# simplew4y/VeritasFi

Hardware: AMD Instinct MI355X
Metric: queries/sec top-100 over 10Mx768 corpus (higher is better)
Workload: dtype f16

## Files before the change

### veritasfi_amd/csrc/vf_api.hip

```cpp
#include "../../include/veritasfi_hip.h"
#include "vf_internal.h"
#include "vf_route.h"

#include <fcntl.h>
#include <float.h>
#include <sys/stat.h>
#include <unistd.h>
#include <math.h>
#include <string.h>

#include <algorithm>
#include <atomic>
#include <mutex>
#include <string>
#include <vector>

using namespace vf;

static thread_local std::string g_err;

static int fail(int code, const std::string& msg) {
    g_err = msg;
    return code;
}
// ... 106 lines not shown
    int nq = 0, k = 0;
    int64_t* d_ids = nullptr; float* d_scores = nullptr;
    hipStream_t user = nullptr;
};

}

struct vf_index {
    int device = 0;
    int64_t n = 0;
    int64_t cap = 0;
    int d = 0, dp = 0, dtype = 0;
    int64_t id_offset = 0;
    int n_cu = 256;
    int64_t aux_applied = -1;
    bool owns_rows = false;
    void* rows_orig = nullptr;
    void* rows_scan = nullptr;
    bool owns_scan = false;
    float* norm = nullptr;
    float* inv_scan = nullptr;
    float* cn_cache = nullptr;
    unsigned char* rows_img = nullptr;
    bool owns_img = false;
    float* inv_img = nullptr;
    float rho_max = 0.0f;
    float rho_mean = 0.0f;
    bool image_refused = false;
    float rho_sum = 0.0f;
    std::mutex mu;
    Slot slots[kSlots];
    int64_t force_path = -1, sample_rows = -1, margin = -1, cap_opt = 0, waves_opt = 0, scan_g = 0,
            refresh_every = 128, debug = 0, steal_opt = 0, wide_opt = 1, wide_sync = -1, wide_mfma = -1, wide8_waves = 8, wide8_stage = 0,
            aux_cus = -1, sample_grid = -1, overlap_scans = -1, scan_impl = 2, sample_impl = -1, scan_image = 1, wide_rows = 1, image_mfma = -1;
    vf_search_stats stats{};
    bool profile = false;
    double prof_scan_ms = 0.0, prof_pipe_ms = 0.0;
    int64_t prof_launches = 0, prof_bytes = 0;
    hipEvent_t ev_span = nullptr;
    bool span_started = false;
    bool span_slot[4] = {false, false, false, false};
    DevBuf st_q, st_ids, st_sc;
    DevBuf st_add, st_rho;
    std::vector<vf_index*> shards;
    std::vector<int> peer_ok;
    GroupSlot gslots[kSlots];
};

static int ensure_pinned(Slot& s, size_t nq_total) {
    if (nq_total <= s.h_cap) return VF_OK;
    if (s.h_flags) (void)hipHostFree(s.h_flags);
    if (s.h_counts) (void)hipHostFree(s.h_counts);
    s.h_flags = nullptr; s.h_counts = nullptr; s.h_cap = 0;
    size_t cap = std::max<size_t>(nq_total, 256);
    VF_HIP(hipHostMalloc((void**)&s.h_flags, cap * sizeof(int), hipHostMallocMapped));
    VF_HIP(hipHostMalloc((void**)&s.h_counts, cap * sizeof(u32), hipHostMallocMapped));
    VF_HIP(hipHostGetDevicePointer((void**)&s.d_flags, s.h_flags, 0));
    VF_HIP(hipHostGetDevicePointer((void**)&s.d_counts, s.h_counts, 0));
    s.h_cap = cap;
    return VF_OK;
}

static int build_image(vf_index* ix, int64_t mode);

static bool known_dtype(int64_t dtype) { return dtype >= VF_DTYPE_F32 && dtype <= VF_DTYPE_INT8; }
static size_t dtype_bytes(int dtype) { return dtype == VF_DTYPE_F32 ? 4 : (dtype == VF_DTYPE_F16 ? 2 : 1); }

static RouteIn route_in(const vf_index* ix, const Slot* s = nullptr) {
    RouteIn in;
    in.n = ix->n; in.d = ix->d; in.dp = ix->dp; in.dtype = ix->dtype; in.n_cu = ix->n_cu;
    in.has_scan = ix->rows_scan && ix->inv_scan;
    in.has_image = ix->rows_img != nullptr; in.rho_mean = ix->rho_mean;
    in.group = !ix->shards.empty();
    in.aux_applied = ix->aux_applied;
    in.masked = s && s->scan_stream && s->scan_stream != s->stream;
    in.force_path = ix->force_path; in.wide = ix->wide_opt; in.wide_mfma = ix->wide_mfma; in.wide8_waves = ix->wide8_waves;
    in.wide8_stage = ix->wide8_stage; in.wide_rows = ix->wide_rows; in.scan_impl = ix->scan_impl; in.sample_impl = ix->sample_impl;
    in.sample_grid = ix->sample_grid; in.steal = ix->steal_opt; in.scan_image = ix->scan_image; in.image_mfma = ix->image_mfma;
    in.aux_cus = ix->aux_cus; in.overlap_scans = ix->overlap_scans; in.margin = ix->margin; in.cap = ix->cap_opt; in.waves = ix->waves_opt;
    in.sample_rows = ix->sample_rows; in.debug = ix->debug;
    return in;
}

static int build_common(vf_index* ix) {
    hipDeviceProp_t prop;
    VF_HIP(hipGetDeviceProperties(&prop, ix->device));
    ix->n_cu = prop.multiProcessorCount > 0 ? prop.multiProcessorCount : 256;
    VF_HIP(scan_configure());
    const int dt = ix->dtype;
    const size_t scan_esz = byte_rows(dt) ? 1 : 2;
    ix->dp = (ix->d + 127) / 128 * 128;
    ix->cap = ix->n;
    const size_t npad = (size_t)ix->cap + 64;
    VF_HIP(hipMalloc((void**)&ix->norm, npad * sizeof(float)));
    VF_HIP(hipMalloc((void**)&ix->inv_scan, npad * sizeof(float)));
    VF_HIP(hipMemset(ix->norm, 0, npad * sizeof(float)));
    VF_HIP(hipMemset(ix->inv_scan, 0, npad * sizeof(float)));
    const bool need_scan = ix->n > kSmallN;
    void* scan_out = nullptr;
    if (need_scan) {
        if (dt != VF_DTYPE_F32 && ix->dp == ix->d && ((uintptr_t)ix->rows_orig % 16) == 0) {
            ix->rows_scan = ix->rows_orig;
            ix->owns_scan = false;
        } else {
            VF_HIP(hipMalloc((void**)&ix->rows_scan, (size_t)ix->cap * ix->dp * scan_esz));
            ix->owns_scan = true;
            scan_out = ix->rows_scan;
        }
    }
    VF_HIP(launch_prep_rows(ix->rows_orig, dt, ix->n, ix->d, ix->dp, scan_out, ix->norm, ix->inv_scan, nullptr));
    VF_TRY(build_image(ix, ix->scan_image));
    if (ix->n > 0 && ix->n <= kSmallN) {
        VF_HIP(hipMalloc((void**)&ix->cn_cache, (size_t)std::min<int64_t>(ix->cap, kSmallN) * ix->d * sizeof(float)));
// ... 574 lines not shown
    else if (s == "wide8_waves") {
#ifdef VF_EXPERIMENTS
        if (value != 4 && value != 8) return fail(VF_EINVAL, "wide8_waves must be 8 (one 512-thread workgroup per CU, 256-query tiles: the default) or 4 (two 256-thread workgroups, 128-query tiles: measured slower, DESIGN.md 4)");
#else
        if (value != 8) return fail(VF_EINVAL, "wide8_waves must be 8 (the 4-wave form was measured slower and is built with -DVF_EXPERIMENTS only: DESIGN.md 4)");
#endif
        ix->wide8_waves = value;
    }
    else if (s == "wide_mfma") { if (!in_range(-1, 1)) return fail(VF_EINVAL, "wide_mfma must be -1 (auto: the fp8 instruction for e4m3 rows), 0 (fp16 matrix instruction on converted rows) or 1 (the fp8 instruction on the e4m3 row bytes: k_scan_wide8)"); ix->wide_mfma = value; }
    else if (s == "wide_sync") { if (!in_range(-1, 8)) return fail(VF_EINVAL, "wide_sync must be -1 (off) or a slack of 0..8 super-tiles"); ix->wide_sync = value; }
    else if (s == "aux_cus") {
        if (!in_range(-1, 128)) return fail(VF_EINVAL, "aux_cus must be -1 (auto) or in [0, 128]");
        if (ix->aux_applied >= 0 && value != ix->aux_cus)
            return fail(VF_EINVAL, "aux_cus is fixed once the first search has created the scan streams: set it before searching");
        ix->aux_cus = value;
    }
    else if (s == "sample_grid") { if (!in_range(-1, 1024)) return fail(VF_EINVAL, "sample_grid must be -1 (auto), 0 (one workgroup per range) or a workgroup count"); ix->sample_grid = value; }
    else if (s == "scan_impl") { if (!in_range(1, 5)) return fail(VF_EINVAL, "scan_impl must be 1 (k_scan), 2 (auto: k_scan2 for fp16 rows, k_scan2r where it measured faster), 3 (k_scan2 wherever it fits, e4m3 rows converted), 4 (k_scan2 for fp16 rows, never k_scan2r) or 5 (k_scan2r wherever a shape of it exists: fp16 rows of 384 / 512 / 768 / 1024 elements, e4m3 rows of 768 / 1024)"); ix->scan_impl = value; }
    else if (s == "sample_impl") { if (!in_range(-1, 1)) return fail(VF_EINVAL, "sample_impl must be -1 (auto: k_scan2r's operand path for the sample pass where it exists and the CU split is on), 0 (k_scan) or 1 (k_scan2r wherever it fits)"); ix->sample_impl = value; }
    else if (s == "overlap_scans") { if (!in_range(-1, 1)) return fail(VF_EINVAL, "overlap_scans must be -1 (auto), 0 or 1"); ix->overlap_scans = value; }
    else if (s == "scan_image") {
        if (!in_range(0, 2)) return fail(VF_EINVAL, "scan_image must be 0 (off), 1 (auto: when it fits with headroom) or 2 (force)");
        if (!ix->shards.empty()) { ix->scan_image = value; return VF_OK; }
        for (const Slot& sl : ix->slots) if (sl.pending) return fail(VF_EINVAL, "scan_image cannot change while a search is pending");
        DeviceGuard restore_callers_device;
        VF_HIP(hipSetDevice(ix->device));
        VF_HIP(hipDeviceSynchronize());
        ix->image_refused = false;
        if (value == 0) free_image(ix);
        else VF_TRY(build_image(ix, value));
        ix->scan_image = value;
    }
    else if (s == "image_mfma") { if (!in_range(-1, 2)) return fail(VF_EINVAL, "image_mfma must be -1 (auto), 0 (the int8 row image on the fp16 matrix instruction, fp16 queries), 1 (on the int8 matrix instruction, the queries as one int8 plane) or 2 (as two planes, hi + lo: the band of 0)"); ix->image_mfma = value; }
    else if (s == "wide_rows") { if (!in_range(0, 2)) return fail(VF_EINVAL, std::string("wide_rows must be 0 (rows of more than 2432 padded elements never take the fused path), 1 (auto: from ") + std::to_string(kWideRowsMinRows) + " rows, e4m3 rows from " + std::to_string(kWideRowsMinRows8) + ", int8 rows from " + std::to_string(kWideRowsMinRowsI8) + ") or 2 (wherever k_scan_ksplit / k_scan_ksplit8 serve them; int8 rows: from " + std::to_string(kWideRowsMinRowsI8) + " rows)"); ix->wide_rows = value; }
    else if (s == "debug") ix->debug = value;
    else if (s == "profile") {
        ix->profile = value != 0; ix->prof_scan_ms = ix->prof_pipe_ms = 0.0; ix->prof_launches = 0;
        ix->span_started = false;
        for (bool& b : ix->span_slot) b = false;
    }
    else return fail(VF_EINVAL, "vf_index_set_option: unknown option " + s);
    return VF_OK;
}

static int exact_search(vf_index* ix, Slot& s, const float* qn_dev, int nq, int k, int64_t* out_ids,
                        float* out_scores, hipStream_t st) {
    const int dt = ix->dtype;
    const int64_t chunk = kSmallN;
    const int64_t nchunks = ix->n == 0 ? 1 : (ix->n + chunk - 1) / chunk;
    if (nchunks > 1) {
        int64_t P = 1;
        while (P < 2 * (int64_t)k) P <<= 1;
        if (P * 8 > 160 * 1024) return fail(VF_EUNSUPPORTED, "exact chunked search supports k <= 8192 when n > 16384");
    }
    VF_TRY(s.dense_s.ensure((size_t)nq * chunk * sizeof(float)));
    if (nchunks == 1) {
        const float* cn = ix->cn_cache;
        if (!cn && ix->n > 0) {
            VF_TRY(s.cn_tmp.ensure((size_t)chunk * ix->d * sizeof(float)));
            VF_HIP(launch_normalize_rows(ix->rows_orig, dt, 0, ix->n, ix->d, ix->norm, s.cn_tmp.as<float>(), st));
            cn = s.cn_tmp.as<float>();
        }
        VF_HIP(launch_dense_dot16(qn_dev, nq, cn, ix->n, ix->d, s.dense_s.as<float>(), chunk, st));
        VF_HIP(launch_sort_rows(s.dense_s.as<float>(), chunk, nq, (int)ix->n, k, ix->id_offset, (long long*)out_ids,
                                out_scores, k, st));
        return VF_OK;
// ... 168 lines not shown
        s.timed = ix->profile;
        if (s.timed) VF_HIP(hipEventRecord(s.ev_t[2], st));
        for (int b0 = 0; b0 < nq; b0 += bl) {
            const int nb = std::min(bl, nq - b0);
            VF_TRY(wide_pass(ix, s, in, p, d_queries + (size_t)b0 * ix->d, nb, k, d_ids + (size_t)b0 * k, d_scores + (size_t)b0 * k,
                             b0, s.qn.as<float>() + (size_t)b0 * ix->d, s.timed && b0 == 0, st, slot_id));
            ++s.wide_launches; s.wide_queries += nb;
        }
        if (s.timed) VF_HIP(hipEventRecord(s.ev_t[3], st));
        VF_HIP(hipEventRecord(s.ev_done, st));
        return VF_OK;
    }
    VF_TRY(s.s0.ensure((size_t)kMaxBatch * p.total_waves * p.samp * sizeof(float)));
    VF_TRY(s.cnt.ensure((size_t)kMaxBatch * kCntStride * sizeof(u32)));
    VF_TRY(s.tau.ensure(kMaxBatch * sizeof(int)));
    VF_TRY(s.hist.ensure((size_t)kMaxBatch * kHistBins * sizeof(u32)));
    VF_TRY(s.hist_coarse.ensure((size_t)kMaxBatch * 64 * sizeof(u32)));
    VF_TRY(s.cand.ensure((size_t)kMaxBatch * p.cap * sizeof(u64)));
    VF_TRY(s.tilecnt.ensure((size_t)p.grid * sizeof(u32)));
    s.timed = ix->profile;
    if (s.timed) VF_HIP(hipEventRecord(s.ev_t[2], st));
    if (s.wgbase_n != ix->n || s.wgbase_grid != p.grid) {
        std::vector<long long> base(p.grid);
        for (int w = 0; w < p.grid; ++w) base[w] = ix->n * (long long)w / p.grid;
        VF_TRY(s.wgbase.ensure((size_t)p.grid * sizeof(long long)));
        VF_HIP(hipMemcpy(s.wgbase.p, base.data(), (size_t)p.grid * sizeof(long long), hipMemcpyHostToDevice));
        s.wgbase_n = ix->n; s.wgbase_grid = p.grid;
    }
    for (int b0 = 0; b0 < nq; b0 += bl) {
        const int nb = std::min(bl, nq - b0);
        const BatchRoute b = route_batch(in, r, nb);
        const int qt = b.tile;
        float* qn_b = s.qn.as<float>() + (size_t)b0 * ix->d;
        VF_HIP(launch_prep_queries(d_queries + (size_t)b0 * ix->d, nb, ix->d, ix->dp, qt, qn_b, s.image_i8 ? nullptr : s.qimg.as<_Float16>(), st));
        ScanArgs a{};
        a.rows = (const char*)ix->rows_scan; a.inv_scan = ix->inv_scan; a.qimg = s.qimg.as<_Float16>();
        if (s.image_i8) {
            VF_TRY(s.qimg8.ensure((size_t)ix->dp * kMaxBatch * 2));
            VF_TRY(s.epsq.ensure(kMaxBatch * sizeof(float)));
            VF_TRY(s.qscale.ensure(kMaxBatch * sizeof(float)));
            VF_TRY(s.bandq.ensure(2 * kMaxBatch * sizeof(int)));
            VF_HIP(launch_prep_q8(qn_b, nb, ix->d, ix->dp, qt, s.image_i8, (signed char*)s.qimg8.p, s.qscale.as<float>(), s.epsq.as<float>(), s.bandq.as<int>(),
                                  p.eps, p.tau_band, p.fine_band, st));
            a.qimg = (const _Float16*)s.qimg8.p; a.q_scale = s.qscale.as<float>(); a.band_q = s.bandq.as<int>();
        }
        a.n = ix->n; a.dp = ix->dp; a.row_bytes = (long long)ix->dp * (byte_rows(ix->dtype) ? 1 : 2); a.total_waves = p.total_waves; a.samp = p.samp;
        if (p.image) { a.rows = (const char*)ix->rows_img; a.inv_scan = ix->inv_img; a.off_scan = image_offsets(ix); a.row_bytes = ix->dp; }
        a.s0 = s.s0.as<float>(); a.wg_base = s.wgbase.as<long long>(); a.cnt = s.cnt.as<u32>(); a.tau_bin = s.tau.as<int>(); a.hist = s.hist.as<u32>();
        a.cand = s.cand.as<u64>(); a.cap = p.cap; a.kprime = p.kprime; a.tau_band = p.tau_band;
        a.hist_coarse = s.hist_coarse.as<u32>(); a.stage_cap = b.stage_cap;
        a.tile_cnt = ix->steal_opt ? s.tilecnt.as<u32>() : nullptr; a.scan_grid = p.grid;
        a.dbg = nullptr;
        if (ix->debug & 128) { VF_TRY(s.dbg.ensure((size_t)p.total_waves * ((ix->debug & 512) ? 72 : 4) * sizeof(u64))); a.dbg = s.dbg.as<u64>(); if (ix->debug & 512) VF_HIP(hipMemsetAsync(s.dbg.p, 0, s.dbg.bytes, st)); }
        a.refresh_every = (int)std::min<int64_t>(256, std::max<int64_t>(4, std::max<int64_t>(1, ix->refresh_every) * nb / kMaxBatch));
        while (a.refresh_every & (a.refresh_every - 1)) a.refresh_every &= a.refresh_every - 1;
        a.nq = nb; a.debug = (int)ix->debug;
        if (ix->n / p.total_waves < p.samp)
            VF_HIP(hipMemsetAsync(a.s0, 0xFF, (size_t)qt * p.total_waves * p.samp * sizeof(float), st));
        switch (b.sample) {
        case kKernelKsplit: VF_HIP(launch_scan_ksplit(a, kModeSample, b.sample_grid, st)); break;
        case kKernelKsplit8: VF_HIP(launch_scan_ksplit8(a, kModeSample, b.sample_grid, b.sample_rows, st)); break;
        case kKernelScan2r: {
            ScanArgs as = a;
            as.stage_cap = 0;
            VF_HIP(launch_scan2r_sample(as, qt, b.sample_grid, b.sample_rows, st));
            break;
        }
        default: VF_HIP(launch_scan(a, kModeSample, qt, b.sample_grid, (int)ix->scan_g, b.sample_rows, st));
        }
        VF_HIP(launch_sel0(a, qt, st));
        hipStream_t sst = s.scan_stream;
        if (sst != st) {
            VF_HIP(hipEventRecord(s.ev_pro, st));
            VF_HIP(hipStreamWaitEvent(sst, s.ev_pro, 0));
        }
        if (!route_overlap(in))
// ... 790 lines not shown
```

### veritasfi_amd/csrc/vf_internal.h

```cpp
#pragma once
#include <hip/hip_runtime.h>
#include <math.h>
#include <stdint.h>

#include "../../include/veritasfi_hip.h"

#include <string>

#include "vf_ksplit_geom.h"

namespace vf {

int set_error(int code, const std::string& msg);

typedef unsigned long long u64;
typedef unsigned int u32;

struct DeviceGuard {
    int prev = -1;
    DeviceGuard() { if (hipGetDevice(&prev) != hipSuccess) prev = -1; }
    ~DeviceGuard() { if (prev >= 0) (void)hipSetDevice(prev); }
    DeviceGuard(const DeviceGuard&) = delete;
    DeviceGuard& operator=(const DeviceGuard&) = delete;
};
// ... 109 lines not shown
    unsigned char* img;
    float* inv_img; float* off_img;
    u32* rho_max_bits; float* rho_sum;
};
hipError_t launch_append_rows(const AppendArgs& a, hipStream_t s);
hipError_t launch_prep_queries(const float* q, int nq, int d, int dp, int qn_tile ,
                               float* qn, _Float16* qimg, hipStream_t s);
hipError_t launch_normalize_rows(const void* rows, int dt , long long row0, long long nrows, int d,
                                 const float* norm, float* out, hipStream_t s);
hipError_t launch_normalize_rows_gather(const void* rows, int dt, const long long* sel , int nsel, int d,
                                        const float* norm, float* out, hipStream_t s);
hipError_t launch_dense_dot16(const float* qn, int nq, const float* cn, long long nrows, int d,
                              float* out, long long out_stride, hipStream_t s);
hipError_t launch_sort_rows(const float* scores, long long score_stride, int nq, int n, int k,
                            long long id_base, long long* out_ids, float* out_scores, int out_stride,
                            hipStream_t s);
hipError_t launch_scan(const ScanArgs& a, int mode, int qn_tile, int grid, int want_g ,
                       RowForm rows , hipStream_t s);
hipError_t launch_rebias_i8(const void* in, void* out, long long bytes, hipStream_t s);
hipError_t launch_debug_cvt_e4m3(const unsigned char* in, float* out, int count, hipStream_t s);
hipError_t launch_debug_mfma_i8(const signed char* A, const signed char* B, int* C, hipStream_t s);
hipError_t launch_scan2(const ScanArgs& a, int qn_tile, int grid, RowForm rows , hipStream_t s);
hipError_t launch_scan2r(const ScanArgs& a, int qn_tile, int grid, RowForm rows, hipStream_t s);
hipError_t launch_scan2r_sample(const ScanArgs& a, int qn_tile, int grid, RowForm rows, hipStream_t s);
hipError_t launch_scan_ksplit(const ScanArgs& a, int mode, int grid, hipStream_t s);
hipError_t launch_scan_ksplit8(const ScanArgs& a, int mode, int grid, RowForm rows, hipStream_t s);
hipError_t launch_scan_wide(const ScanArgs& a, int mode, RowForm rows , hipStream_t s);
hipError_t launch_prep_wide8(const float* qn, int nq, int d, int dp, int qtot, unsigned char* img8, float* eps_q, hipStream_t s);
hipError_t launch_scan_wide8(const ScanArgs& a, int waves , hipStream_t s);
int scan_wide8_occupancy(int waves, int stage_cap);
hipError_t launch_prep_q8(const float* qn, int nq, int d, int dp, int qn_tile, int planes , signed char* img8, float* q_scale, float* eps_q, int* band_q,
                          float eps_img, int tau_band, int fine_band, hipStream_t s);
hipError_t launch_sel0(const ScanArgs& a, int qn_tile, hipStream_t s);
hipError_t launch_final(FinalArgs a, int nq, hipStream_t s);
hipError_t launch_merge_topk(const long long* ids_parts, const float* score_parts, int nparts, int nq,
                             int k, long long* ids, float* scores, hipStream_t s);
hipError_t launch_merge_topk_packed(const void* parts, int nparts, int nq, int k, long long* ids, float* scores,
                                    hipStream_t s);
hipError_t launch_fuse_rank(const float* a, const float* b, int n, float* out, long long* order,
                            hipStream_t s);
inline long long packed_part_bytes(int nq, int k) { return ((long long)nq * k * 12 + 15) / 16 * 16; }
hipError_t scan_configure();

}
```

### veritasfi_amd/csrc/vf_kernels.hip

```cpp
#include "vf_internal.h"

#include <float.h>
#include <algorithm>
#include <type_traits>

#include <mutex>

namespace vf {

typedef _Float16 h8 __attribute__((ext_vector_type(8)));
typedef _Float16 h4 __attribute__((ext_vector_type(4)));
typedef float f16v __attribute__((ext_vector_type(16)));
typedef int i4v __attribute__((ext_vector_type(4)));
typedef int i16v __attribute__((ext_vector_type(16)));
typedef int i8v __attribute__((ext_vector_type(8)));

__device__ __forceinline__ float group16_tree(float acc) {
    acc = acc + __shfl_down(acc, 8, 16);
    acc = acc + __shfl_down(acc, 4, 16);
    acc = acc + __shfl_down(acc, 2, 16);
    acc = acc + __shfl_down(acc, 1, 16);
    return acc;
}

// ... 211 lines not shown
    const int slot = blockIdx.x;
    const int tid = threadIdx.x;
    if (slot < nq) {
        const float* x = q + (long long)slot * d;
        for (int j = tid; j < d; j += 256) xs[j] = x[j];
        __syncthreads();
        if (tid < 16) {
            float acc = 0.0f;
            for (int j = tid; j < d; j += 16) acc = __builtin_fmaf(xs[j], xs[j], acc);
            acc = group16_tree(acc);
            if (tid == 0) s_norm = canon_norm_from_sumsq(acc);
        }
        __syncthreads();
        const float inv = canon_inv(s_norm);
        for (int j = tid; j < dp; j += 256) {
            float v = 0.0f;
            if (j < d) {
                v = xs[j] * inv;
                qn[(long long)slot * d + j] = v;
            }
            if (qimg) qimg[((long long)(j >> 3) * QN + slot) * 8 + (j & 7)] = (_Float16)v;
        }
    } else if (qimg) {
        for (int j = tid; j < dp; j += 256) qimg[((long long)(j >> 3) * QN + slot) * 8 + (j & 7)] = (_Float16)0.0f;
    }
}

hipError_t launch_prep_queries(const float* q, int nq, int d, int dp, int qn_tile, float* qn, _Float16* qimg,
                               hipStream_t s) {
    hipLaunchKernelGGL(k_prep_queries, dim3(qn_tile), dim3(256), (size_t)d * sizeof(float), s, q, nq, d, dp, qn_tile, qn, qimg);
    return hipGetLastError();
}

__global__ __launch_bounds__(256) void k_prep_q8(const float* qn, int nq, int d, int dp, int QN, int planes, signed char* img8, float* q_scale,
                                                  float* eps_q, int* band_q, float eps_img, int tau_band, int fine_band) {
    __shared__ float red_f[256];
    __shared__ double red_d[256];
    const int slot = blockIdx.x, tid = threadIdx.x;
    const bool live = slot < nq;
    float mx = 0.0f;
    if (live) for (int j = tid; j < d; j += 256) mx = fmaxf(mx, fabsf(qn[(long long)slot * d + j]));
    red_f[tid] = mx;
    __syncthreads();
    for (int o = 128; o; o >>= 1) { if (tid < o) red_f[tid] = fmaxf(red_f[tid], red_f[tid + o]); __syncthreads(); }
    mx = red_f[0];
    bool finite = mx <= FLT_MAX;
    const float sc = (finite && mx > 0.0f) ? mx / 127.0f : 1.0f;
    const float sc2 = sc / 254.0f;
    double res = 0.0;
    for (int j = tid; j < dp; j += 256) {
        float code = 0.0f, lo = 0.0f;
        if (live && j < d) {
            const float x = qn[(long long)slot * d + j];
            code = fminf(fmaxf(rintf(x / sc), -127.0f), 127.0f);
            double dx = (double)x - (double)sc * (double)code;
            if (planes == 2) {
                lo = fminf(fmaxf(rintf((float)dx / sc2), -127.0f), 127.0f);
                dx -= (double)sc2 * (double)lo;
            }
            res += dx * dx;
        }
        const long long at = (((long long)(j >> 4) * planes) * QN + slot) * 16 + (j & 15);
        img8[at] = (signed char)(int)code;
        if (planes == 2) img8[at + (long long)QN * 16] = (signed char)(int)lo;
    }
    red_d[tid] = res;
    __syncthreads();
    for (int o = 128; o; o >>= 1) { if (tid < o) red_d[tid] += red_d[tid + o]; __syncthreads(); }
    if (tid == 0) {
        const double rd = sqrt(red_d[0]);
        float rho = (float)rd;
        if ((double)rho < rd) rho = nextafterf(rho, INFINITY);
        if (!finite || !(rd <= (double)FLT_MAX)) rho = INFINITY;
        const Q8Bound b = image_q8_bound(live ? rho : 0.0f);
        q_scale[slot] = live ? (planes == 2 ? sc2 : sc) : 0.0f;
        eps_q[slot] = image_q8_eps(eps_img, b.eps_add);
        band_q[slot] = tau_band + b.tau_bins;
        band_q[QN + slot] = fine_band + b.fine_bins;
    }
}

hipError_t launch_prep_q8(const float* qn, int nq, int d, int dp, int qn_tile, int planes, signed char* img8, float* q_scale, float* eps_q, int* band_q,
                          float eps_img, int tau_band, int fine_band, hipStream_t s) {
    hipLaunchKernelGGL(k_prep_q8, dim3(qn_tile), dim3(256), 0, s, qn, nq, d, dp, qn_tile, planes, img8, q_scale, eps_q, band_q, eps_img, tau_band, fine_band);
    return hipGetLastError();
}

__device__ __forceinline__ float normalised_elem(float x, float nm) { return x * canon_inv(nm); }

__global__ __launch_bounds__(256) void k_normalize_rows(const void* rows, int dt, long long row0,
                                                         long long nrows, int d, const float* norm, float* out) {
    const long long total = nrows * (long long)d;
    for (long long i = (long long)blockIdx.x * 256 + threadIdx.x; i < total; i += (long long)gridDim.x * 256) {
        const long long r = i / d;
        out[i] = normalised_elem(load_elem(rows, dt, (row0 + r) * (long long)d + (i - r * d)), norm[row0 + r]);
    }
}

hipError_t launch_normalize_rows(const void* rows, int dt, long long row0, long long nrows, int d,
                                 const float* norm, float* out, hipStream_t s) {
    if (nrows <= 0) return hipSuccess;
    long long blocks = (nrows * (long long)d + 255) / 256;
    if (blocks > 65536) blocks = 65536;
    hipLaunchKernelGGL(k_normalize_rows, dim3((unsigned)blocks), dim3(256), 0, s, rows, dt, row0, nrows, d, norm,
                       out);
    return hipGetLastError();
}

__global__ __launch_bounds__(256) void k_append_rows(AppendArgs a) {
    __shared__ u32 wg_max;
    __shared__ float wg_sum;
    const bool stats = a.img != nullptr;
// ... 1828 lines not shown
                        if constexpr (PLANES == 2) { v = v * 254.0f + (float)acci[1][nt][e]; acci[1][nt][e] = 0; }
                        acc[nt][e] = v * sq[nt];
                        acci[0][nt][e] = 0;
                    }
            }
            epi.sync_tau = sync_now;
            if (sync_now) {
#pragma unroll
                for (int nt = 0; nt < NT; ++nt) epi.tau_g[nt] = *(const int*)(sc + (nt * kQueryTile + r31) * 4);
            }
            tile_epilogue<NT, MODE, true, true, F8 >= 2>(a, acc, epi, t0, t_hi, t_s0, lane, ctl);
#pragma unroll
            for (int nt = 0; nt < NT; ++nt)
#pragma unroll
                for (int e = 0; e < 16; ++e) acc[nt][e] = 0.0f;
            VF_PC(pt1 = cyc(); pc_epi += pt1 - pt0)
            ++tiles_done;
            if (!more) break;
            cur_tile = nxt;
            src_cur = src_nxt;
        }
    }
    if (dbg && dbg_rec > 4) dbg[69] = (unsigned long long)tiles_done;
    asm volatile("s_waitcnt vmcnt(0)" ::: "memory");
    if (MODE == kModeSample) return;
    if (lane == 0) atomicAdd((u32*)(ctl + 8), 1u);
    if (dbg) dbg[1] = wall_clock64();
    __syncthreads();
    if (dbg) dbg[2] = wall_clock64();
    {
        const u32 staged = *(const u32*)ctl;
        const u32 nst = staged < (u32)a.stage_cap ? staged : (u32)a.stage_cap;
        uint4* ent = (uint4*)(ctl + kCtlBytes);
        u32* qcnt = (u32*)(kImgBytes ? img : smem);
        u32* qbase = qcnt + QN;
        if (tid < QN) qcnt[tid] = 0u;
        __syncthreads();
        for (u32 i = tid; i < nst; i += THREADS) {
            const uint4 e = ent[i];
            const u32 q = e.z & 0xFFu;
            if (e.w != 1u || q >= (u32)QN) continue;
            ent[i].w = 2u + atomicAdd(qcnt + q, 1u);
        }
        __syncthreads();
        if (tid < QN) {
            const u32 c = qcnt[tid];
            qbase[tid] = c ? atomicAdd(a.cnt + tid * kCntStride, c) : 0u;
        }
        __syncthreads();
        for (u32 i = tid; i < nst; i += THREADS) {
            const uint4 e = ent[i];
            if (e.w < 2u) continue;
            const u32 q = e.z & 0xFFu;
            const u32 gs = qbase[q] + (e.w - 2u);
            if (gs < (u32)a.cap) a.cand[(long long)q * a.cap + gs] = ((u64)e.y << 32) | (u64)e.x;
        }
    }
    if (dbg && dbg_rec > 4) dbg[71] = __builtin_amdgcn_s_memtime() - c_entry;
#ifdef VF_EXPERIMENTS
    if (dbg && dbg_rec > 4 && prof) { dbg[4] = pc_wait; dbg[5] = pc_use; dbg[6] = pc_fill; dbg[7] = pc_head; dbg[8] = pc_epi; dbg[9] = pc_n; }
#endif
#undef VF_PC
    if (dbg) dbg[3] = wall_clock64();
}

constexpr int kWideNT = kWideQ / kQueryTile, kWideRows = 256;
// ... 1065 lines not shown
        if (rows_are_fp8) hipLaunchKernelGGL((k_scan2<1, 1>), dim3(grid), dim3(kScan2Threads), lds, s, a);
        else hipLaunchKernelGGL((k_scan2<1, 0>), dim3(grid), dim3(kScan2Threads), lds, s, a);
    } else {
        if (rows_are_fp8) hipLaunchKernelGGL((k_scan2<2, 1>), dim3(grid), dim3(kScan2Threads), lds, s, a);
        else hipLaunchKernelGGL((k_scan2<2, 0>), dim3(grid), dim3(kScan2Threads), lds, s, a);
    }
    return hipGetLastError();
}

#define VF_SCAN2R_PRODUCT(X, NT, MODE) X(NT, MODE, 0, 12, 6, 6, 1) X(NT, MODE, 0, 16, 6, 4, 1) X(NT, MODE, 0, 8, 4, 6, 1) X(NT, MODE, 0, 6, 3, 6, 1) X(NT, MODE, 1, 6, 3, 6, 1) X(NT, MODE, 1, 8, 3, 4, 1) \
    X(NT, MODE, 2, 6, 3, 6, 1) X(NT, MODE, 3, 6, 6, 6, 1) X(NT, MODE, 4, 6, 3, 6, 1)
#ifdef VF_EXPERIMENTS
#define VF_SCAN2R_SHAPES(X, NT, MODE) VF_SCAN2R_PRODUCT(X, NT, MODE) X(NT, MODE, 0, 12, 6, 6, 0) X(NT, MODE, 1, 6, 3, 4, 1)
#else
#define VF_SCAN2R_SHAPES(X, NT, MODE) VF_SCAN2R_PRODUCT(X, NT, MODE)
#endif
#define VF_SCAN2R_ALL(X) VF_SCAN2R_SHAPES(X, 1, kModeMain) VF_SCAN2R_SHAPES(X, 2, kModeMain) VF_SCAN2R_SHAPES(X, 1, kModeSample) VF_SCAN2R_SHAPES(X, 2, kModeSample)
static hipError_t launch_scan2r_any(const ScanArgs& a, int qn_tile, int mode, int grid, RowForm f8, size_t lds, hipStream_t s) {
    Scan2rShape sh = scan2r_shape(a.dp, f8);
#ifdef VF_EXPERIMENTS
    if (f8 == 1 && a.dp == 768 && (a.debug & 2048)) sh.RING = 4;
#endif
    const int nt = qn_tile / kQueryTile;
    bool done = false;
    const int ar = (!f8 && a.dp == 768 && (a.debug & 1024)) ? 0 : 1;
#define VF_X(NT, MODE, F8, S_, RB_, RING_, AR_) \
    if (!done && nt == NT && mode == MODE && f8 == F8 && sh.S == S_ && sh.RB == RB_ && sh.RING == RING_ && ar == AR_) { \
        hipLaunchKernelGGL((k_scan2r<NT, MODE, F8, S_, RB_, RING_, AR_>), dim3(grid), dim3(kScan2Waves * 64), lds, s, a); done = true; }
    VF_SCAN2R_ALL(VF_X)
#undef VF_X
    return done ? hipGetLastError() : hipErrorInvalidValue;
}
hipError_t launch_scan2r(const ScanArgs& a, int qn_tile, int grid, RowForm f8, hipStream_t s) {
    return launch_scan2r_any(a, qn_tile, kModeMain, grid, f8, scan2r_lds_bytes(a.dp, qn_tile, a.stage_cap, f8), s);
}
hipError_t launch_scan2r_sample(const ScanArgs& a, int qn_tile, int grid, RowForm f8, hipStream_t s) {
    return launch_scan2r_any(a, qn_tile, kModeSample, grid, f8, scan2r_lds_bytes(a.dp, qn_tile, 0, f8), s);
}

template <int NT, int G, int MODE>
static hipError_t configure_one() {
    hipError_t e = hipFuncSetAttribute((const void*)k_scan<NT, G, MODE, 0>, hipFuncAttributeMaxDynamicSharedMemorySize,
                                       160 * 1024);
    if (e != hipSuccess) return e;
    e = hipFuncSetAttribute((const void*)k_scan<NT, G, MODE, 2>, hipFuncAttributeMaxDynamicSharedMemorySize, 160 * 1024);
    if (e != hipSuccess) return e;
    return hipFuncSetAttribute((const void*)k_scan<NT, G, MODE, 1>, hipFuncAttributeMaxDynamicSharedMemorySize, 160 * 1024);
}

__device__ __forceinline__ int wave_tau_from_lds(const u32* lh, int kprime, int lane) {
    u32 hv[32];
    u32 sum = 0;
#pragma unroll
    for (int i = 0; i < 32; ++i) { hv[i] = lh[lane * 32 + i]; sum += hv[i]; }
    u32 suf = sum;
#pragma unroll
    for (int off = 1; off < 64; off <<= 1) {
        const u32 v = __shfl_down(suf, off);
        if (lane + off < 64) suf += v;
    }
    const u32 above = suf - sum;
    int best = -1;
    if (above < (u32)kprime && suf >= (u32)kprime) {
        u32 run = above;
        bool found = false;
#pragma unroll
// ... 457 lines not shown
```

### veritasfi_amd/csrc/vf_route.h

```cpp
#pragma once
#include <math.h>
#include <stdint.h>

#include <algorithm>

#include "../../include/veritasfi_hip.h"
#include "vf_ksplit_geom.h"

namespace vf {

struct RouteIn {
    int64_t n = 0;
    int d = 0, dp = 0, dtype = 0, n_cu = 256;
    bool has_scan = false;
    bool has_image = false;
    float rho_mean = 0.0f;
    bool group = false;
    int64_t aux_applied = -1;
    bool masked = false;
    int64_t force_path = -1, wide = 1, wide_mfma = -1, wide8_waves = 8, wide8_stage = 0, wide_rows = 1, scan_impl = 2, sample_impl = -1,
            sample_grid = -1, steal = 0, scan_image = 1, image_mfma = -1, aux_cus = -1, overlap_scans = -1, margin = -1, cap = 0, waves = 0,
            sample_rows = -1, debug = 0;
};

enum ScanKernel : int {
    kKernelNone = 0, kKernelScan = 1, kKernelScan2 = 2, kKernelWide = 3, kKernelWide8 = 4, kKernelScan2r = 5, kKernelKsplit = 6,
    kKernelKsplit8 = 7,
};

struct FusedPlan {
    int kprime, cap, total_waves, grid, samp;
    float eps;
    bool image;
    int tau_band, fine_band;
};

struct SearchRoute {
    int path = 2;
    int per_pass = kMaxBatch;
    bool wide = false;
    bool image = false;
    int planes = 0;
    FusedPlan plan{};
};

struct BatchRoute {
    int tile;
    ScanKernel sample;
    int sample_grid;
    RowForm sample_rows;
    ScanKernel main;
    RowForm main_rows;
    int stage_cap;
};

// ... 99 lines not shown
    int margin = in.margin >= 0 ? (int)in.margin : std::max(24, k / 4);
    const double u16 = 1.0 / 2048.0;
    const float eps_plan = (float)(u16 * (in.dtype == VF_DTYPE_F32 ? 2.0 : 1.0) + sqrt((double)in.d) * ldexp(1.0, -24) +
                                   2.0 * in.d * ldexp(1.0, -24) + 1e-6);
    if (in.margin < 0 && ksplit_width(in.dp)) {
        const double z = sqrt(2.0 * log(std::max(3.0, (double)in.n / k)));
        margin = std::max(margin, (int)ceil(2.5 * eps_plan * k * z * sqrt((double)in.d)));
    }
    p.kprime = in.margin >= 0 ? k + margin : (k + margin + 31) / 32 * 32;
    p.kprime = std::min(p.kprime, 4096);
    int cap = kMaxCap;
    while (cap < 4 * p.kprime && cap < 16384) cap <<= 1;
    if (in.cap > 0) { cap = 1; while (cap < in.cap) cap <<= 1; cap = std::min(cap, 16384); }
    while (cap < 2 * p.kprime) cap <<= 1;
    p.cap = cap;
    const int64_t scan_cus = in.n_cu - route_aux_cus(in);
    int64_t wgs = std::min<int64_t>(scan_cus, std::max<int64_t>(1, in.n / 512));
    if (in.waves > 0) wgs = std::max<int64_t>(1, in.waves / (kScanThreads / 64));
    p.grid = (int)wgs;
    p.total_waves = p.grid * (kScanThreads / 64);
    p.samp = in.sample_rows > 0 ? (int)in.sample_rows : ((in.n <= 1500000 && 8ll * p.total_waves >= 16ll * p.kprime) ? 8 : 16);
    if (in.cap <= 0) {
        const double sample_rows = (double)p.total_waves * p.samp;
        const double expect = p.kprime * (1.0 + log(std::max(1.0, (double)in.n / std::max(1.0, sample_rows))));
        while (p.cap < (int)(1.6 * expect) && p.cap < 32768) p.cap <<= 1;
    }
    p.eps = eps_plan;
    if (image) {
        image_bound(in.d, in.dtype, in.rho_mean, &p.eps, &p.tau_band, &p.fine_band);
        p.kprime = k;
        p.cap = 32768;
    }
    return p;
}

constexpr int kWideMinQueries = 129;
constexpr int kWideMinQueries16 = 65;
constexpr int kWideMinQueriesKsplit = 33;
constexpr int kWideMinQueriesKsplit8 = 65;
constexpr int kWideMaxQueries = 1024;
constexpr int kWideTile = kWideQ;
inline bool wide_possible(const RouteIn& in, int nq) {
    const bool ks = ksplit_width(in.dp);
    if (in.wide == 0 || nq < (in.wide > 1 ? (int)in.wide : ks ? (byte_rows(in.dtype) ? kWideMinQueriesKsplit8 : kWideMinQueriesKsplit) : (byte_rows(in.dtype) ? kWideMinQueries : kWideMinQueries16))) return false;
    return in.dp % (byte_rows(in.dtype) ? 256 : 128) == 0;
}

inline WidePass route_wide_pass(const RouteIn& in, const FusedPlan& p, int nb) {
    WidePass w;
    w.qtot = (nb + kWideTile - 1) / kWideTile * kWideTile;
    w.jtiles = w.qtot / kWideTile;
    w.rgroups = std::max(1, in.n_cu / w.jtiles);
    w.cap = p.cap;
    if (p.kprime > 256) w.cap = std::max(w.cap, 16384);
    const bool w8 = (in.wide_mfma > 0 || (in.wide_mfma < 0 && !ksplit_width(in.dp))) && in.dtype == VF_DTYPE_FP8_E4M3 && in.dp % 64 == 0 &&
                    (in.n / w.rgroups + 2 * 256) * (int64_t)in.dp < (int64_t)0xFFFFFFFFll;
    if (w8) {
        if (p.kprime > 256) w.cap = std::max(w.cap, 32768);
    }
    w.main = w8 ? kKernelWide8 : kKernelWide;
    w.rows = stored_rows(in.dtype);
    w.samp = w.jtiles >= 2 ? 64 : 32;
    w.waves = in.wide8_waves == 4 ? 4 : 8;
    w.main_jtiles = w8 && w.waves == 4 ? (nb + 127) / 128 : w.jtiles;
    w.stage_cap = !w8 ? kWideStageCap
                      : in.wide8_stage > 0 ? (int)std::min<int64_t>(in.wide8_stage, scan_wide8_stage_cap(w.waves)) : scan_wide8_stage_cap(w.waves);
// ... 20 lines not shown
    const int qt = b.tile = qn_tile_for(nb);
    const bool ks = ksplit_width(in.dp);
    const int64_t steal = in.steal, scan_impl = in.scan_impl;
    const bool f8rows = in.dtype == VF_DTYPE_FP8_E4M3 || p.image;
    const bool i8conv = in.dtype == VF_DTYPE_INT8 && !p.image;
    const bool r_f8_auto = f8rows && scan_impl == 2 && in.n > kScan2rMinRows && !steal && scan2r_auto_width(in.dp, true);
    const bool sample_r = p.image || (!i8conv && in.sample_impl != 0 && scan_impl != 1 && scan2r_stage_cap(in.dp, qt, f8rows ? kRowsE4m3 : kRowsF16) >= kStageMinEntries &&
                          (in.sample_impl == 1 || (!f8rows && in.masked && scan2r_auto_width(in.dp, false)) || r_f8_auto));
    if (ks) {
        b.sample = byte_rows(in.dtype) ? kKernelKsplit8 : kKernelKsplit;
        b.sample_grid = p.grid;
        b.sample_rows = stored_rows(in.dtype);
    } else if (sample_r) {
        const int64_t sg_r = in.sample_grid > 0 ? in.sample_grid : (in.masked ? route_aux_cus(in) : p.grid);
        b.sample = kKernelScan2r;
        b.sample_grid = (int)std::min<int64_t>(std::max<int64_t>(sg_r, 1), p.grid);
        b.sample_rows = p.image ? image_rows(r.planes) : (f8rows ? kRowsE4m3 : kRowsF16);
    } else {
        const int64_t sg_opt = in.sample_grid >= 0 ? in.sample_grid : (in.masked ? 4 * route_aux_cus(in) : 0);
        b.sample = kKernelScan;
        b.sample_grid = sg_opt > 0 ? (int)std::min<int64_t>(sg_opt, p.grid) : p.grid;
        b.sample_rows = stored_rows(in.dtype);
    }
    const RowForm f8 = in.dtype == VF_DTYPE_FP8_E4M3 ? kRowsE4m3 : kRowsF16;
    if (ks) {
        b.main = byte_rows(in.dtype) ? kKernelKsplit8 : kKernelKsplit;
        b.main_rows = stored_rows(in.dtype);
        b.stage_cap = ksplit_stage_cap(in);
        return b;
    }
    if (p.image) {
        b.main = kKernelScan2r;
        b.main_rows = image_rows(r.planes);
        b.stage_cap = scan2r_stage_cap(in.dp, qt, b.main_rows);
        return b;
    }
    const int cap2 = i8conv ? 0 : (((scan_impl == 3 || ((scan_impl == 2 || scan_impl == 4 || scan_impl == 5) && !f8)) && !steal) ? scan2_stage_cap(in.dp, qt, f8) : 0);
    const bool r_auto = scan_impl == 2 && in.n > kScan2rMinRows && scan2r_auto_width(in.dp, f8 != 0) && (f8 || (in.masked && route_overlap(in)));
#ifdef VF_EXPERIMENTS
    const bool dbg_r = f8 || !(in.debug & (32 | 64));
#else
    const bool dbg_r = true;
#endif
    const int capr = ((scan_impl == 5 || r_auto) && !steal && dbg_r && !i8conv) ? scan2r_stage_cap(in.dp, qt, f8) : 0;
    if (capr >= kStageMinEntries) {
        b.main = kKernelScan2r; b.main_rows = f8; b.stage_cap = capr;
    } else if (cap2 >= kStageMinEntries) {
        b.main = kKernelScan2; b.main_rows = f8; b.stage_cap = cap2;
    } else {
        b.main = kKernelScan; b.main_rows = stored_rows(in.dtype); b.stage_cap = scan_stage_cap(in.dp, qt);
    }
    return b;
}

}
```

### veritasfi_amd/csrc/vf_scan_lds.h

```cpp
#pragma once
#include <stddef.h>

#if defined(__HIPCC__)
#define VF_HD __host__ __device__ __forceinline__
#else
#define VF_HD inline
#endif

namespace vf {

constexpr int kQueryTile = 32;
constexpr int kMaxBatch = 64;
constexpr int kRowTile = 32;
constexpr int kScanThreads = 512;
constexpr int kHistBins = 2048;
constexpr int kSmallN = 16384;
constexpr int kMaxCap = 8192;
constexpr int kCntStride = 32;
constexpr int kMaxKFused = 2048;

constexpr int kLdsBytes = 160 * 1024;
constexpr int kStageMaxBytes = 32 * 1024;
constexpr int kStageMinEntries = 256;

enum RowForm : int {
    kRowsF16 = 0,
    kRowsE4m3 = 1,
    kRowsI8 = 2,
    kRowsI8Mfma1 = 3,
    kRowsI8Mfma2 = 4,
};
VF_HD bool row_form_bytes(RowForm f) { return f != kRowsF16; }

constexpr int kCtlBytes = 272;

VF_HD int stage_entries(size_t fixed) {
    const size_t freeb = fixed < (size_t)kLdsBytes ? (size_t)kLdsBytes - fixed : 0;
    return (int)((freeb < (size_t)kStageMaxBytes ? freeb : (size_t)kStageMaxBytes) / 16);
}

VF_HD size_t scan_lds_bytes(int dp, int qn_tile) { return (size_t)dp * qn_tile * 2 + kCtlBytes; }
VF_HD int scan_stage_cap(int dp, int qn_tile) { return stage_entries(scan_lds_bytes(dp, qn_tile)); }

constexpr int kScan2Waves = 4, kRing = 3, kSegBytes = 4096, kScratchBytes = 1024;

VF_HD size_t scan2_lds_bytes(int dp, int qn_tile, int stage_cap) {
    const size_t img = (size_t)dp * qn_tile * 2;
    return img + (size_t)kScan2Waves * (kRing * kSegBytes + kScratchBytes) + kCtlBytes + (size_t)stage_cap * 16;
}
VF_HD int scan2_stage_cap(int dp, int qn_tile, RowForm rows) {
    const size_t fixed = scan2_lds_bytes(dp, qn_tile, 0);
    if ((dp >> (rows ? 7 : 6)) < kRing) return 0;
    if (fixed + kStageMinEntries * 16 > (size_t)kLdsBytes) return 0;
    return stage_entries(fixed);
}

struct Scan2rShape { int S, RB, RING; };
VF_HD Scan2rShape scan2r_shape(int dp, RowForm f8) {
    if (!f8 && dp == 768) return {12, 6, 6};
    if (!f8 && dp == 1024) return {16, 6, 4};
    if (!f8 && dp == 512) return {8, 4, 6};
    if (!f8 && dp == 384) return {6, 3, 6};
    if (f8 == kRowsI8Mfma1) return dp == 768 ? Scan2rShape{6, 6, 6} : Scan2rShape{0, 0, 0};
    if (f8 == kRowsI8Mfma2) return dp == 768 ? Scan2rShape{6, 3, 6} : Scan2rShape{0, 0, 0};
    if (f8 && dp == 768) return {6, 3, 6};
    if (f8 && dp == 1024) return {8, 3, 4};
    return {0, 0, 0};
}
VF_HD size_t scan2r_lds_bytes(int dp, int qn_tile, int stage_cap, RowForm f8) {
    const Scan2rShape sh = scan2r_shape(dp, f8);
    const size_t seg_img = (size_t)(f8 ? 128 : 64) * qn_tile * 2;
    return (size_t)(sh.S - sh.RB) * seg_img + (size_t)kScan2Waves * (sh.RING * kSegBytes + kScratchBytes) + kCtlBytes + (size_t)stage_cap * 16;
}
VF_HD int scan2r_stage_cap(int dp, int qn_tile, RowForm f8) {
    if (scan2r_shape(dp, f8).S == 0) return 0;
    const size_t fixed = scan2r_lds_bytes(dp, qn_tile, 0, f8);
    if (fixed + kStageMinEntries * 16 > (size_t)kLdsBytes) return 0;
    return stage_entries(fixed);
}

constexpr int kWideQ = 256, kWideKC = 64;
constexpr int kWideBuf = (kWideKC / 8) * kWideQ * 16;
constexpr int kWideCtl = 16 + 3 * kWideQ * 4;
constexpr int kWideStageCap = 3584;

VF_HD size_t scan_wide_lds_bytes(int stage_cap) { return (size_t)3 * kWideBuf + kWideCtl + (size_t)stage_cap * 16; }
VF_HD size_t scan_wide8_lds_bytes(int waves, int stage_cap) {
    return waves == 8 ? scan_wide_lds_bytes(stage_cap) : (size_t)65536 + (16 + 3 * 128 * 4) + (size_t)stage_cap * 16;
}
VF_HD int scan_wide8_stage_cap(int waves) { return waves == 8 ? kWideStageCap : 896; }

}
```

Measured before the change: 47970.

## Fuse query normalisation into int8 query prep and lift image-scan stage cap

```diff
diff --git a/veritasfi_amd/csrc/vf_api.hip b/veritasfi_amd/csrc/vf_api.hip
--- a/veritasfi_amd/csrc/vf_api.hip
+++ b/veritasfi_amd/csrc/vf_api.hip
@@ -162,7 +162,7 @@
     Slot slots[kSlots];
     int64_t force_path = -1, sample_rows = -1, margin = -1, cap_opt = 0, waves_opt = 0, scan_g = 0,
             refresh_every = 128, debug = 0, steal_opt = 0, wide_opt = 1, wide_sync = -1, wide_mfma = -1, wide8_waves = 8, wide8_stage = 0,
-            aux_cus = -1, sample_grid = -1, overlap_scans = -1, scan_impl = 2, sample_impl = -1, scan_image = 1, wide_rows = 1, image_mfma = -1;
+            aux_cus = -1, sample_grid = -1, overlap_scans = -1, scan_impl = 2, sample_impl = -1, scan_image = 1, wide_rows = 1, image_mfma = -1, image_stage = -1;
     vf_search_stats stats{};
     bool profile = false;
     double prof_scan_ms = 0.0, prof_pipe_ms = 0.0;
@@ -208,7 +208,7 @@
     in.wide8_stage = ix->wide8_stage; in.wide_rows = ix->wide_rows; in.scan_impl = ix->scan_impl; in.sample_impl = ix->sample_impl;
     in.sample_grid = ix->sample_grid; in.steal = ix->steal_opt; in.scan_image = ix->scan_image; in.image_mfma = ix->image_mfma;
     in.aux_cus = ix->aux_cus; in.overlap_scans = ix->overlap_scans; in.margin = ix->margin; in.cap = ix->cap_opt; in.waves = ix->waves_opt;
-    in.sample_rows = ix->sample_rows; in.debug = ix->debug;
+    in.sample_rows = ix->sample_rows; in.debug = ix->debug; in.image_stage = ix->image_stage;
     return in;
 }
 
@@ -849,6 +849,7 @@
         ix->scan_image = value;
     }
     else if (s == "image_mfma") { if (!in_range(-1, 2)) return fail(VF_EINVAL, "image_mfma must be -1 (auto), 0 (the int8 row image on the fp16 matrix instruction, fp16 queries), 1 (on the int8 matrix instruction, the queries as one int8 plane) or 2 (as two planes, hi + lo: the band of 0)"); ix->image_mfma = value; }
+    else if (s == "image_stage") { if (!in_range(-1, 1)) return fail(VF_EINVAL, "image_stage must be -1 (auto: the int8-instruction image scans stage what the LDS leaves where a workgroup's expected share of the candidates exceeds 2048 entries), 0 (2048 entries at most) or 1 (what the LDS leaves, wherever the form has room)"); ix->image_stage = value; }
     else if (s == "wide_rows") { if (!in_range(0, 2)) return fail(VF_EINVAL, std::string("wide_rows must be 0 (rows of more than 2432 padded elements never take the fused path), 1 (auto: from ") + std::to_string(kWideRowsMinRows) + " rows, e4m3 rows from " + std::to_string(kWideRowsMinRows8) + ", int8 rows from " + std::to_string(kWideRowsMinRowsI8) + ") or 2 (wherever k_scan_ksplit / k_scan_ksplit8 serve them; int8 rows: from " + std::to_string(kWideRowsMinRowsI8) + " rows)"); ix->wide_rows = value; }
     else if (s == "debug") ix->debug = value;
     else if (s == "profile") {
@@ -1083,7 +1084,7 @@
         const BatchRoute b = route_batch(in, r, nb);
         const int qt = b.tile;
         float* qn_b = s.qn.as<float>() + (size_t)b0 * ix->d;
-        VF_HIP(launch_prep_queries(d_queries + (size_t)b0 * ix->d, nb, ix->d, ix->dp, qt, qn_b, s.image_i8 ? nullptr : s.qimg.as<_Float16>(), st));
+        if (!s.image_i8) VF_HIP(launch_prep_queries(d_queries + (size_t)b0 * ix->d, nb, ix->d, ix->dp, qt, qn_b, s.qimg.as<_Float16>(), st));
         ScanArgs a{};
         a.rows = (const char*)ix->rows_scan; a.inv_scan = ix->inv_scan; a.qimg = s.qimg.as<_Float16>();
         if (s.image_i8) {
@@ -1091,8 +1092,8 @@
             VF_TRY(s.epsq.ensure(kMaxBatch * sizeof(float)));
             VF_TRY(s.qscale.ensure(kMaxBatch * sizeof(float)));
             VF_TRY(s.bandq.ensure(2 * kMaxBatch * sizeof(int)));
-            VF_HIP(launch_prep_q8(qn_b, nb, ix->d, ix->dp, qt, s.image_i8, (signed char*)s.qimg8.p, s.qscale.as<float>(), s.epsq.as<float>(), s.bandq.as<int>(),
-                                  p.eps, p.tau_band, p.fine_band, st));
+            VF_HIP(launch_prep_queries_q8(d_queries + (size_t)b0 * ix->d, nb, ix->d, ix->dp, qt, qn_b, s.image_i8, (signed char*)s.qimg8.p, s.qscale.as<float>(),
+                                          s.epsq.as<float>(), s.bandq.as<int>(), p.eps, p.tau_band, p.fine_band, st));
             a.qimg = (const _Float16*)s.qimg8.p; a.q_scale = s.qscale.as<float>(); a.band_q = s.bandq.as<int>();
         }
         a.n = ix->n; a.dp = ix->dp; a.row_bytes = (long long)ix->dp * (byte_rows(ix->dtype) ? 1 : 2); a.total_waves = p.total_waves; a.samp = p.samp;
diff --git a/veritasfi_amd/csrc/vf_internal.h b/veritasfi_amd/csrc/vf_internal.h
--- a/veritasfi_amd/csrc/vf_internal.h
+++ b/veritasfi_amd/csrc/vf_internal.h
@@ -165,6 +165,8 @@
 hipError_t launch_prep_q8(const float* qn, int nq, int d, int dp, int qn_tile, int planes , signed char* img8, float* q_scale, float* eps_q, int* band_q,
                           float eps_img, int tau_band, int fine_band, hipStream_t s);
 hipError_t launch_sel0(const ScanArgs& a, int qn_tile, hipStream_t s);
+hipError_t launch_prep_queries_q8(const float* q, int nq, int d, int dp, int qn_tile, float* qn, int planes, signed char* img8, float* q_scale,
+                                  float* eps_q, int* band_q, float eps_img, int tau_band, int fine_band, hipStream_t s);
 hipError_t launch_final(FinalArgs a, int nq, hipStream_t s);
 hipError_t launch_merge_topk(const long long* ids_parts, const float* score_parts, int nparts, int nq,
                              int k, long long* ids, float* scores, hipStream_t s);
diff --git a/veritasfi_amd/csrc/vf_kernels.hip b/veritasfi_amd/csrc/vf_kernels.hip
--- a/veritasfi_amd/csrc/vf_kernels.hip
+++ b/veritasfi_amd/csrc/vf_kernels.hip
@@ -267,14 +267,13 @@
     return hipGetLastError();
 }
 
-__global__ __launch_bounds__(256) void k_prep_q8(const float* qn, int nq, int d, int dp, int QN, int planes, signed char* img8, float* q_scale,
-                                                  float* eps_q, int* band_q, float eps_img, int tau_band, int fine_band) {
+__device__ __forceinline__ void prep_q8_slot(const float* x, bool live, int slot, int d, int dp, int QN, int planes, signed char* img8, float* q_scale,
+                                             float* eps_q, int* band_q, float eps_img, int tau_band, int fine_band) {
     __shared__ float red_f[256];
     __shared__ double red_d[256];
-    const int slot = blockIdx.x, tid = threadIdx.x;
-    const bool live = slot < nq;
+    const int tid = threadIdx.x;
     float mx = 0.0f;
-    if (live) for (int j = tid; j < d; j += 256) mx = fmaxf(mx, fabsf(qn[(long long)slot * d + j]));
+    if (live) for (int j = tid; j < d; j += 256) mx = fmaxf(mx, fabsf(x[j]));
     red_f[tid] = mx;
     __syncthreads();
     for (int o = 128; o; o >>= 1) { if (tid < o) red_f[tid] = fmaxf(red_f[tid], red_f[tid + o]); __syncthreads(); }
@@ -286,9 +285,9 @@
     for (int j = tid; j < dp; j += 256) {
         float code = 0.0f, lo = 0.0f;
         if (live && j < d) {
-            const float x = qn[(long long)slot * d + j];
-            code = fminf(fmaxf(rintf(x / sc), -127.0f), 127.0f);
-            double dx = (double)x - (double)sc * (double)code;
+            const float xj = x[j];
+            code = fminf(fmaxf(rintf(xj / sc), -127.0f), 127.0f);
+            double dx = (double)xj - (double)sc * (double)code;
             if (planes == 2) {
                 lo = fminf(fmaxf(rintf((float)dx / sc2), -127.0f), 127.0f);
                 dx -= (double)sc2 * (double)lo;
@@ -313,6 +312,48 @@
         band_q[slot] = tau_band + b.tau_bins;
         band_q[QN + slot] = fine_band + b.fine_bins;
     }
+}
+
+__global__ __launch_bounds__(256) void k_prep_q8(const float* qn, int nq, int d, int dp, int QN, int planes, signed char* img8, float* q_scale,
+                                                  float* eps_q, int* band_q, float eps_img, int tau_band, int fine_band) {
+    const int slot = blockIdx.x;
+    prep_q8_slot(qn + (long long)slot * d, slot < nq, slot, d, dp, QN, planes, img8, q_scale, eps_q, band_q, eps_img, tau_band, fine_band);
+}
+
+__global__ __launch_bounds__(256) void k_prep_queries_q8(const float* q, int nq, int d, int dp, int QN, float* qn, int planes, signed char* img8,
+                                                          float* q_scale, float* eps_q, int* band_q, float eps_img, int tau_band, int fine_band) {
+    extern __shared__ __attribute__((aligned(16))) char smem_raw[];
+    float* xs = (float*)smem_raw;
+    __shared__ float s_norm;
+    const int slot = blockIdx.x, tid = threadIdx.x;
+    const bool live = slot < nq;
+    if (live) {
+        const float* x = q + (long long)slot * d;
+        for (int j = tid; j < d; j += 256) xs[j] = x[j];
+        __syncthreads();
+        if (tid < 16) {
+            float acc = 0.0f;
+            for (int j = tid; j < d; j += 16) acc = __builtin_fmaf(xs[j], xs[j], acc);
+            acc = group16_tree(acc);
+            if (tid == 0) s_norm = canon_norm_from_sumsq(acc);
+        }
+        __syncthreads();
+        const float inv = canon_inv(s_norm);
+        for (int j = tid; j < d; j += 256) {
+            const float v = xs[j] * inv;
+            qn[(long long)slot * d + j] = v;
+            xs[j] = v;
+        }
+    }
+    __syncthreads();
+    prep_q8_slot(xs, live, slot, d, dp, QN, planes, img8, q_scale, eps_q, band_q, eps_img, tau_band, fine_band);
+}
+
+hipError_t launch_prep_queries_q8(const float* q, int nq, int d, int dp, int qn_tile, float* qn, int planes, signed char* img8, float* q_scale,
+                                  float* eps_q, int* band_q, float eps_img, int tau_band, int fine_band, hipStream_t s) {
+    hipLaunchKernelGGL(k_prep_queries_q8, dim3(qn_tile), dim3(256), (size_t)d * sizeof(float), s, q, nq, d, dp, qn_tile, qn, planes, img8, q_scale, eps_q,
+                       band_q, eps_img, tau_band, fine_band);
+    return hipGetLastError();
 }
 
 hipError_t launch_prep_q8(const float* qn, int nq, int d, int dp, int qn_tile, int planes, signed char* img8, float* q_scale, float* eps_q, int* band_q,
@@ -2207,6 +2248,7 @@
         const u32 staged = *(const u32*)ctl;
         const u32 nst = staged < (u32)a.stage_cap ? staged : (u32)a.stage_cap;
         uint4* ent = (uint4*)(ctl + kCtlBytes);
+        if (dbg && dbg_rec > 4) dbg[69] |= (unsigned long long)(staged - nst) << 32;
         u32* qcnt = (u32*)(kImgBytes ? img : smem);
         u32* qbase = qcnt + QN;
         if (tid < QN) qcnt[tid] = 0u;
@@ -3338,6 +3380,7 @@
     return done ? hipGetLastError() : hipErrorInvalidValue;
 }
 hipError_t launch_scan2r(const ScanArgs& a, int qn_tile, int grid, RowForm f8, hipStream_t s) {
+    if (a.stage_cap < 0 || scan2r_lds_bytes(a.dp, qn_tile, a.stage_cap, f8) > (size_t)kLdsBytes) return hipErrorInvalidValue;
     return launch_scan2r_any(a, qn_tile, kModeMain, grid, f8, scan2r_lds_bytes(a.dp, qn_tile, a.stage_cap, f8), s);
 }
 hipError_t launch_scan2r_sample(const ScanArgs& a, int qn_tile, int grid, RowForm f8, hipStream_t s) {
diff --git a/veritasfi_amd/csrc/vf_route.h b/veritasfi_amd/csrc/vf_route.h
--- a/veritasfi_amd/csrc/vf_route.h
+++ b/veritasfi_amd/csrc/vf_route.h
@@ -20,7 +20,7 @@
     bool masked = false;
     int64_t force_path = -1, wide = 1, wide_mfma = -1, wide8_waves = 8, wide8_stage = 0, wide_rows = 1, scan_impl = 2, sample_impl = -1,
             sample_grid = -1, steal = 0, scan_image = 1, image_mfma = -1, aux_cus = -1, overlap_scans = -1, margin = -1, cap = 0, waves = 0,
-            sample_rows = -1, debug = 0;
+            sample_rows = -1, debug = 0, image_stage = -1;
 };
 
 enum ScanKernel : int {
@@ -186,6 +186,22 @@
         p.cap = 32768;
     }
     return p;
+}
+
+constexpr int kImageQ8TypicalBins = 9;
+inline double image_share_estimate(const RouteIn& in, const FusedPlan& p, int planes, int nb) {
+    const int k = std::max(1, p.kprime);
+    const double w = (double)(p.tau_band + (planes == 1 ? kImageQ8TypicalBins : 0)) / (kHistBins / 2);
+    const double z = sqrt(2.0 * log(std::max(3.0, (double)in.n / k)));
+    const double in_band = k * exp(std::min(20.0, z * sqrt((double)in.d) * w));
+    const double sample_rows = std::max(1.0, (double)p.total_waves * p.samp);
+    const double per_list = 1.6 * in_band * (1.0 + log(std::max(1.0, (double)in.n / sample_rows)));
+    return per_list * nb / std::max(1, p.grid);
+}
+inline bool image_stage_lifted(const RouteIn& in, const FusedPlan& p, int planes, int nb) {
+    if (!p.image || !scan2r_stage_liftable(image_rows(planes)) || in.image_stage == 0) return false;
+    if (in.image_stage > 0) return true;
+    return in.n >= kImageMinRows && image_share_estimate(in, p, planes, nb) > (double)(kStageMaxBytes / 16);
 }
 
 constexpr int kWideMinQueries = 129;
@@ -272,7 +288,7 @@
     if (p.image) {
         b.main = kKernelScan2r;
         b.main_rows = image_rows(r.planes);
-        b.stage_cap = scan2r_stage_cap(in.dp, qt, b.main_rows);
+        b.stage_cap = scan2r_stage_cap(in.dp, qt, b.main_rows, image_stage_lifted(in, p, r.planes, nb));
         return b;
     }
     const int cap2 = i8conv ? 0 : (((scan_impl == 3 || ((scan_impl == 2 || scan_impl == 4 || scan_impl == 5) && !f8)) && !steal) ? scan2_stage_cap(in.dp, qt, f8) : 0);
diff --git a/veritasfi_amd/csrc/vf_scan_lds.h b/veritasfi_amd/csrc/vf_scan_lds.h
--- a/veritasfi_amd/csrc/vf_scan_lds.h
+++ b/veritasfi_amd/csrc/vf_scan_lds.h
@@ -34,9 +34,9 @@
 
 constexpr int kCtlBytes = 272;
 
-VF_HD int stage_entries(size_t fixed) {
+VF_HD int stage_entries(size_t fixed, size_t max_bytes = (size_t)kStageMaxBytes) {
     const size_t freeb = fixed < (size_t)kLdsBytes ? (size_t)kLdsBytes - fixed : 0;
-    return (int)((freeb < (size_t)kStageMaxBytes ? freeb : (size_t)kStageMaxBytes) / 16);
+    return (int)((freeb < max_bytes ? freeb : max_bytes) / 16);
 }
 
 VF_HD size_t scan_lds_bytes(int dp, int qn_tile) { return (size_t)dp * qn_tile * 2 + kCtlBytes; }
@@ -72,11 +72,12 @@
     const size_t seg_img = (size_t)(f8 ? 128 : 64) * qn_tile * 2;
     return (size_t)(sh.S - sh.RB) * seg_img + (size_t)kScan2Waves * (sh.RING * kSegBytes + kScratchBytes) + kCtlBytes + (size_t)stage_cap * 16;
 }
-VF_HD int scan2r_stage_cap(int dp, int qn_tile, RowForm f8) {
+VF_HD bool scan2r_stage_liftable(RowForm f8) { return f8 == kRowsI8Mfma1 || f8 == kRowsI8Mfma2; }
+VF_HD int scan2r_stage_cap(int dp, int qn_tile, RowForm f8, bool lifted = false) {
     if (scan2r_shape(dp, f8).S == 0) return 0;
     const size_t fixed = scan2r_lds_bytes(dp, qn_tile, 0, f8);
     if (fixed + kStageMinEntries * 16 > (size_t)kLdsBytes) return 0;
-    return stage_entries(fixed);
+    return stage_entries(fixed, lifted && scan2r_stage_liftable(f8) ? (size_t)kLdsBytes : (size_t)kStageMaxBytes);
 }
 
 constexpr int kWideQ = 256, kWideKC = 64;
```

New measurement: 48710, median of 5. +1.5%, better.
